# isxml/YOLO-SOMI

Measured on AMD Instinct MI355X. Metric: images/sec train (forward+loss+backward+Adam+EMA) @640, VisDrone-shaped synthetic, yolov5l-SOMI (DCNv3 blocks), higher is better.
Workload: dtype f32; 1 GPU; yolov5l-SOMI (DCNv3 blocks) training step: uint8 ingest + forward (batch-stat BN) + ComputeLoss + backward + Adam + EMA, 640x640, batch 32/GPU (BASELINE configs[1] shape); batch_per_gpu=32, imgsz=640, params=77918970, classes=10, parallelism=dp1

## Files before the change

### include/somi_hip.h

```cpp
#ifndef SOMI_HIP_H
#define SOMI_HIP_H

#include <stddef.h>
#include <stdint.h>

#ifdef __cplusplus
extern "C" {
#endif

#define SOMI_ABI_VERSION 15

#define SOMI_EINVAL   (-1)
#define SOMI_ENOTIMPL (-2)
#define SOMI_EWORKSPACE (-3)

typedef void *somi_stream_t;

int somi_abi_version(void);
const char *somi_last_error(void);
size_t somi_sizeof_desc(int which);

enum somi_act { SOMI_ACT_NONE = 0, SOMI_ACT_SILU = 1, SOMI_ACT_GELU = 2, SOMI_ACT_RELU = 3, SOMI_ACT_SIGMOID = 4,
                SOMI_ACT_LEAKY = 5 ,
                SOMI_ACT_HSWISH = 6  };
// ... 326 lines not shown

int somi_detect_decode_f32(const float *box, int box_cs, const float *cls, int cls_cs, const float *anchors_px_host,
                           float stride, float *raw, float *z, int B, int ny, int nx, int na, int nc, int total,
                           int row_off, somi_stream_t stream);

int somi_red_nchunk(long npix);
int somi_bn_stats_nhwc_f32(const float *x, int x_cs, int x_coff, long npix, int C, float eps, float momentum,
                           const float *gamma, const float *beta, float *mean, float *rstd, float *scale, float *shift,
                           float *running_mean, float *running_var, float *workspace, somi_stream_t stream);
int somi_bn_stats_act_nhwc_f32(const float *x, int x_cs, int x_coff, int act, long npix, int C, float eps, float momentum,
                               const float *gamma, const float *beta, float *mean, float *rstd, float *scale, float *shift,
                               float *running_mean, float *running_var, float *workspace, somi_stream_t stream);
int somi_bn_stats_partials_f32(const float *part_sum, const float *part_sumsq, int rows, long npix, int C, float eps, float momentum,
                               const float *gamma, const float *beta, float *mean, float *rstd, float *scale, float *shift,
                               float *running_mean, float *running_var, float *workspace, somi_stream_t stream);
int somi_bn_local_sums_f64(const float *x, int x_cs, int x_coff, long npix, int C, const float *pivot , const float *part_sum,
                           const float *part_sumsq, int rows, double *sums, float *workspace, somi_stream_t stream);
int somi_bn_stats_from_sums_f64(const double *all_sums, int nranks, int C, float eps, float momentum, const float *gamma, const float *beta,
                                float *mean, float *rstd, float *scale, float *shift, float *running_mean, float *running_var,
                                somi_stream_t stream);
int somi_bn_act_backward_sums_f64(const float *dz, int dz_cs, int dz_coff, const float *x, int x_cs, int x_coff, const float *mean,
                                  const float *scale, const float *shift, int act, int order, long npix, int C, double *sums, float *workspace,
                                  somi_stream_t stream);
int somi_bn_act_backward_apply_sync_f32(const float *dz, int dz_cs, int dz_coff, const float *x, int x_cs, int x_coff, const float *mean,
                                        const float *rstd, const float *scale, const float *shift, int act, int order,
                                        const double *local_sums, const double *all_sums, int nranks, float *dx, int dx_cs, int dx_coff,
                                        float *dgamma, float *dbeta, long npix, int C, float *workspace, somi_stream_t stream);
int somi_chan_affine_act_nhwc_f32(const float *x, int x_cs, int x_coff, const float *scale, const float *shift, int act,
                                  int order, float *z, int z_cs, int z_coff, long npix, int C, const float *residual ,
                                  int res_cs, int res_coff, somi_stream_t stream);
// ... 55 lines not shown
                        float *db, float *dx, int ldx_out, int dx_accumulate, float *workspace, int B, int nin, int nout,
                        somi_stream_t stream);
int somi_odconv_synth_f32(const float *attn, const float *Wk, const float *biask, float *wout, float *bout, int B, int Cin, int Cin_pad,
                          int Cout, int kk, int K, somi_stream_t stream);
size_t somi_odconv_synth_bwd_workspace_floats(int B, int Cin, int Cout, int kk, int K);
int somi_odconv_synth_bwd_f32(const float *dWb, const float *attn, const float *Wk, const float *biask, const float *dbias_b, float *dWk,
                              float *dbiask, float *dattn, float *workspace, int B, int Cin, int Cin_pad, int Cout, int kk, int K,
                              somi_stream_t stream);

int somi_adam_ema_step_f32(float *param, const float *grad, float *exp_avg, float *exp_avg_sq, float *ema, long n, float lr, float beta1,
                           float beta2, float eps, float weight_decay, int step, float ema_decay, somi_stream_t stream);
int somi_sgd_ema_step_f32(float *param, const float *grad, float *momentum_buf, float *ema, long n, float lr, float momentum,
                          float weight_decay, int step, float ema_decay, somi_stream_t stream);
int somi_axpby_f32(float *y, const float *x, long n, float a, float b, somi_stream_t stream);
int somi_pack_dgrad_weights_f32(const float *w_packed, float *w_dgrad, int Cout, int taps, int Cin, somi_stream_t stream);

int somi_gconv2d_stat_rows(int B, int Ho, int Wo, int Cw);
int somi_gconv2d_nhwc_f32(const float *x, int x_cs, int x_coff, int B, int H, int W, int C1, const float *w, int w_cs, const float *bias,
                          int groups, int k, int stride, float *y, int y_cs, int y_coff, int C2, int Cw, int act, const float *residual,
                          int res_cs, int res_coff, float *stat_sum, float *stat_sumsq, const float *stat_pivot, somi_stream_t stream);
int somi_gconv2d_dgrad_nhwc_f32(const float *dy, int dy_cs, int dy_coff, int B, int Ho, int Wo, int C2, const float *w, int w_cs, int groups,
                                int k, int stride, float *dx, int dx_cs, int dx_coff, int H, int W, int C1, int Cx, const float *acc1,
                                int acc1_cs, int acc1_coff, const float *acc2, int acc2_cs, int acc2_coff, somi_stream_t stream);
size_t somi_gconv2d_wgrad_workspace_floats(int B, int Ho, int Wo, int C2, int cin_g, int k);
int somi_gconv2d_wgrad_nhwc_f32(const float *x, int x_cs, int x_coff, int B, int H, int W, int C1, const float *dy, int dy_cs, int dy_coff,
                                int Ho, int Wo, int C2, int groups, int k, int stride, float *dw, int accumulate, float *workspace,
                                size_t workspace_floats, somi_stream_t stream);

int somi_dwlk_strip_length(void);
int somi_dwlk_strips_per_workgroup(int B, int H, int W, int C, int wgrad);
// ... 162 lines not shown
```

### yolo-somi_amd/csrc/optim.hip

```cpp
#include "common.h"

namespace somi {

typedef float f32x4 __attribute__((ext_vector_type(4)));

__global__ __launch_bounds__(256) void adam_ema_kernel(float *__restrict__ p, const float *__restrict__ g, float *__restrict__ m, float *__restrict__ v,
                                                       float *__restrict__ ema, long n, float lr, float b1, float b2, float eps, float wd,
                                                       float bc1, float bc2_sqrt, float ema_d) {
    const float step = lr / bc1;
    const long n4 = n >> 2;
    for (long i = blockIdx.x * 256L + threadIdx.x; i < n4; i += (long)gridDim.x * 256) {
        f32x4 pv = *reinterpret_cast<f32x4 *>(p + i * 4);
        f32x4 gv = *reinterpret_cast<const f32x4 *>(g + i * 4) + wd * pv;
        f32x4 mv = b1 * *reinterpret_cast<f32x4 *>(m + i * 4) + (1.f - b1) * gv;
        f32x4 vv = b2 * *reinterpret_cast<f32x4 *>(v + i * 4) + (1.f - b2) * gv * gv;
#pragma unroll
        for (int e = 0; e < 4; ++e) pv[e] -= step * mv[e] / (sqrtf(vv[e]) / bc2_sqrt + eps);
        *reinterpret_cast<f32x4 *>(p + i * 4) = pv;
        *reinterpret_cast<f32x4 *>(m + i * 4) = mv;
        *reinterpret_cast<f32x4 *>(v + i * 4) = vv;
        if (ema) *reinterpret_cast<f32x4 *>(ema + i * 4) = ema_d * *reinterpret_cast<f32x4 *>(ema + i * 4) + (1.f - ema_d) * pv;
    }
    for (long i = n4 * 4 + blockIdx.x * 256L + threadIdx.x; i < n; i += (long)gridDim.x * 256) {
        float pv = p[i];
// ... 15 lines not shown
        p[i] = pv;
        buf[i] = bv;
        if (ema) ema[i] = ema_d * ema[i] + (1.f - ema_d) * pv;
    }
}

__global__ __launch_bounds__(256) void axpby_kernel(float *__restrict__ y, const float *__restrict__ x, long n, float a, float b) {
    for (long i = blockIdx.x * 256L + threadIdx.x; i < n; i += (long)gridDim.x * 256) y[i] = a * y[i] + b * x[i];
}

static inline int grid_for(long n) {
    long g = (n / 4 + 255) / 256;
    return (int)(g < 1 ? 1 : (g > 4096 ? 4096 : g));
}

__global__ __launch_bounds__(256) void pack_dgrad_kernel(const float *__restrict__ w, float *__restrict__ wt, int Cout, int T, int Cin) {
    __shared__ float tile[32][33];
    const int t = blockIdx.z, co0 = blockIdx.y * 32, ci0 = blockIdx.x * 32;
    const int tx = threadIdx.x & 31, ty = threadIdx.x >> 5;
    for (int r = ty; r < 32; r += 8) {
        const int co = co0 + r, ci = ci0 + tx;
        tile[r][tx] = (co < Cout && ci < Cin) ? w[((size_t)co * T + t) * Cin + ci] : 0.f;
    }
    __syncthreads();
    for (int r = ty; r < 32; r += 8) {
        const int ci = ci0 + r, co = co0 + tx;
        if (ci < Cin && co < Cout) wt[((size_t)ci * T + t) * Cout + co] = tile[tx][r];
    }
}

}

using namespace somi;

extern "C" int somi_adam_ema_step_f32(float *param, const float *grad, float *exp_avg, float *exp_avg_sq, float *ema, long n, float lr, float beta1,
                                      float beta2, float eps, float weight_decay, int step, float ema_decay, somi_stream_t stream) {
    SOMI_REQUIRE(param && grad && exp_avg && exp_avg_sq && n > 0 && step >= 1, SOMI_EINVAL, "adam: bad arguments");
    SOMI_REQUIRE(aligned16(param) && aligned16(grad) && aligned16(exp_avg) && aligned16(exp_avg_sq) && (!ema || aligned16(ema)), SOMI_EINVAL,
                 "adam: segments must be 16 B aligned");
    const float bc1 = 1.f - powf(beta1, (float)step), bc2 = 1.f - powf(beta2, (float)step);
    hipLaunchKernelGGL(adam_ema_kernel, dim3(grid_for(n)), dim3(256), 0, (hipStream_t)stream, param, grad, exp_avg, exp_avg_sq, ema, n, lr, beta1,
                       beta2, eps, weight_decay, bc1, sqrtf(bc2), ema_decay);
    return launch_status("somi_adam_ema_step_f32");
// ... 8 lines not shown
}

extern "C" int somi_axpby_f32(float *y, const float *x, long n, float a, float b, somi_stream_t stream) {
    SOMI_REQUIRE(y && x && n > 0, SOMI_EINVAL, "axpby: bad arguments");
    hipLaunchKernelGGL(axpby_kernel, dim3(grid_for(n * 4)), dim3(256), 0, (hipStream_t)stream, y, x, n, a, b);
    return launch_status("somi_axpby_f32");
}

extern "C" int somi_pack_dgrad_weights_f32(const float *w_packed, float *w_dgrad, int Cout, int taps, int Cin, somi_stream_t stream) {
    using namespace somi;
    SOMI_REQUIRE(w_packed && w_dgrad && Cout > 0 && taps > 0 && Cin > 0 && taps < 65536, SOMI_EINVAL, "pack dgrad: bad arguments");
    hipLaunchKernelGGL(pack_dgrad_kernel, dim3(cdiv(Cin, 32), cdiv(Cout, 32), taps), dim3(256), 0, (hipStream_t)stream, w_packed, w_dgrad,
                       Cout, taps, Cin);
    return launch_status("somi_pack_dgrad_weights_f32");
}
```

### yolo-somi_amd/csrc/train_ops.hip

```cpp
#include "common.h"

namespace somi {
typedef int i32x4_ __attribute__((ext_vector_type(4)));

typedef float f32x4 __attribute__((ext_vector_type(4)));

static inline int red_chunk(long npix) {
    long c = (npix + 1023) / 1024;
    c = (c + 31) / 32 * 32;
    return (int)(c < 32 ? 32 : (c > 4096 ? 4096 : c));
}

__device__ __forceinline__ float act_fwd(float u, int act) { return apply_act_rt(u, act); }
__device__ __forceinline__ float act_grad(float u, int act) {
    switch (act) {
        case SOMI_ACT_SILU: { const float s = 1.f / (1.f + expf(-u)); return s * (1.f + u * (1.f - s)); }
        case SOMI_ACT_GELU: return 0.5f * (1.f + erff(u * 0.70710678118654752440f)) + u * 0.39894228040143267794f * expf(-0.5f * u * u);
        case SOMI_ACT_RELU: return u > 0.f ? 1.f : 0.f;
        case SOMI_ACT_SIGMOID: { const float s = 1.f / (1.f + expf(-u)); return s * (1.f - s); }
        case SOMI_ACT_LEAKY: return u > 0.f ? 1.f : 0.1f;
        case SOMI_ACT_HSWISH: return u <= -3.f ? 0.f : (u >= 3.f ? 1.f : (2.f * u + 3.f) * (1.f / 6.f));
        default: return 1.f;
    }
}
// ... 21 lines not shown
            for (long p = p0 + rr; p < p1; p += rows_par) f(p, (cq0 + cq) * 4, s1, s2);
        }
        l1[threadIdx.x] = s1;
        l2[threadIdx.x] = s2;
        __syncthreads();
        if (threadIdx.x < ncq) {
            for (int r2 = 1; r2 < rows_par; ++r2) { s1 += l1[r2 * ncq + cq]; s2 += l2[r2 * ncq + cq]; }
            const long o = (long)chunk * C + (cq0 + cq) * 4;
            *reinterpret_cast<f32x4 *>(part1 + o) = s1;
            *reinterpret_cast<f32x4 *>(part2 + o) = s2;
        }
        __syncthreads();
    }
}

constexpr int S2_CH = 4, S2_GRP = 256 / S2_CH;
__device__ __forceinline__ bool stage2_sums(const float *__restrict__ p1, const float *__restrict__ p2, int nchunk, int C, int &c, double &s1, double &s2) {
    __shared__ double l1[256], l2[256];
    const int cl = threadIdx.x % S2_CH, grp = threadIdx.x / S2_CH;
    c = blockIdx.x * S2_CH + cl;
    double a0 = 0.0, a1 = 0.0, b0 = 0.0, b1 = 0.0;
    if (c < C) {
        constexpr int S2_DEEP = 8;
        for (int k = grp; k < nchunk; k += S2_DEEP * S2_GRP) {
            float v[S2_DEEP], w[S2_DEEP];
#pragma unroll
            for (int j = 0; j < S2_DEEP; ++j) {
                const int r = k + j * S2_GRP;
                const bool ok = r < nchunk;
                v[j] = ok ? p1[(long)r * C + c] : 0.f;
                w[j] = (ok && p2) ? p2[(long)r * C + c] : 0.f;
            }
#pragma unroll
            for (int j = 0; j < S2_DEEP; j += 2) { a0 += v[j]; a1 += v[j + 1]; b0 += w[j]; b1 += w[j + 1]; }
        }
    }
    l1[threadIdx.x] = a0 + a1;
    l2[threadIdx.x] = b0 + b1;
    __syncthreads();
    if (grp != 0 || c >= C) return false;
    double t1 = 0.0, t2 = 0.0;
#pragma unroll
    for (int g = 0; g < S2_GRP; ++g) { t1 += l1[g * S2_CH + cl]; t2 += l2[g * S2_CH + cl]; }
    s1 = t1;
    s2 = t2;
    return true;
// ... 26 lines not shown
    double var = q / (double)npix - dm * dm;
    if (var < 0.0) var = 0.0;
    const float rs = (float)(1.0 / sqrt(var + (double)eps));
    mean[c] = (float)m;
    rstd[c] = rs;
    const float g = gamma ? gamma[c] : 1.f, b = beta ? beta[c] : 0.f;
    scale[c] = g * rs;
    shift[c] = b - (float)m * g * rs;
    if (running_mean) {
        const double unb = npix > 1 ? var * (double)npix / (double)(npix - 1) : var;
        running_mean[c] = (1.f - momentum) * running_mean[c] + momentum * (float)m;
        running_var[c] = (1.f - momentum) * running_var[c] + momentum * (float)unb;
    }
}

__global__ __launch_bounds__(256) void rows_fold_kernel(const float *__restrict__ p1, const float *__restrict__ p2, int rows, int C, int per,
                                                        float *__restrict__ o1, float *__restrict__ o2) {
    const int c = blockIdx.y * 256 + threadIdx.x;
    if (c >= C) return;
    const int r0 = blockIdx.x * per, r1 = min(r0 + per, rows);
    float a = 0.f, b = 0.f;
    for (int r = r0; r < r1; ++r) { a += p1[(size_t)r * C + c]; b += p2[(size_t)r * C + c]; }
    o1[(size_t)blockIdx.x * C + c] = a;
    o2[(size_t)blockIdx.x * C + c] = b;
}

__global__ __launch_bounds__(256) void sums_fold_f64_kernel(const float *__restrict__ p1, const float *__restrict__ p2, int nchunk, int C, long npix,
                                                            double *__restrict__ sums, const float *__restrict__ pivot, int central) {
    int c;
    double s1, s2;
    if (blockIdx.x == 0 && threadIdx.x == 0) sums[2 * (size_t)C] = (double)npix;
    if (!stage2_sums(p1, p2, nchunk, C, c, s1, s2)) return;
    if (central) {
        const double dm = s1 / (double)npix;
        double m2 = s2 - s1 * dm;
        sums[c] = (pivot ? (double)pivot[c] : 0.0) + dm;
        sums[(size_t)C + c] = m2 < 0.0 ? 0.0 : m2;
// ... 386 lines not shown
            }
        }
#pragma unroll
        for (int j = 0; j < 7; ++j) {
            lr[threadIdx.x] = acc[j];
            __syncthreads();
            if (threadIdx.x < ncq) {
                f32x4 t = acc[j];
                for (int r2 = 1; r2 < rows_par; ++r2) t += lr[r2 * ncq + cq];
                *reinterpret_cast<f32x4 *>(part + j * plane + row * C + c) = t;
            }
            __syncthreads();
        }
    }
}
__global__ __launch_bounds__(256) void cbam_bn_bwd_stage2(const float *__restrict__ part, int rows, int nimg, int C, int HW, const float *__restrict__ davg,
                                                          const float *__restrict__ dmax, const float *__restrict__ rstd,
                                                          const float *__restrict__ scale, float *__restrict__ coefA, float *__restrict__ coefB,
                                                          float *__restrict__ coefC, float *dgamma, float *dbeta) {
    __shared__ double l1[256], l2[256];
    const int cl = threadIdx.x % S2_CH, grp = threadIdx.x / S2_CH;
    const int c = blockIdx.x * S2_CH + cl;
    const long plane = (long)rows * C;
    const float inv_hw = 1.f / (float)HW;
    double a1 = 0.0, a2 = 0.0;
    if (c < C) {
        for (int k = grp; k < rows; k += 4 * S2_GRP) {
            float v[4][6], ka[4], km[4];
#pragma unroll
            for (int j = 0; j < 4; ++j) {
                const int r = k + j * S2_GRP;
                const bool ok = r < rows;
                const int b = ok ? r / nimg : 0;
#pragma unroll
                for (int q = 0; q < 6; ++q) v[j][q] = ok ? part[(q + 1) * plane + (long)r * C + c] : 0.f;
                ka[j] = ok ? davg[(long)b * C + c] * inv_hw : 0.f;
                km[j] = ok ? dmax[(long)b * C + c] : 0.f;
            }
#pragma unroll
            for (int j = 0; j < 4; ++j) {
                a1 += (double)(v[j][0] + ka[j] * v[j][2] + km[j] * v[j][4]);
                a2 += (double)(v[j][1] + ka[j] * v[j][3] + km[j] * v[j][5]);
            }
        }
    }
    l1[threadIdx.x] = a1;
    l2[threadIdx.x] = a2;
    __syncthreads();
    if (grp != 0 || c >= C) return;
    double s1 = 0.0, s2 = 0.0;
#pragma unroll
    for (int g = 0; g < S2_GRP; ++g) { s1 += l1[g * S2_CH + cl]; s2 += l2[g * S2_CH + cl]; }
    const double rs = rstd[c], sc = scale[c], n = (double)rows / nimg * HW;
    const double D = rs * s2;
    coefA[c] = (float)sc;
    coefB[c] = (float)(-sc * rs * D / n);
    coefC[c] = (float)(-sc * s1 / n);
// ... 182 lines not shown
    SOMI_REQUIRE(!running_mean == !running_var, SOMI_EINVAL, "bn stats: running_mean and running_var go together");
    hipStream_t s = (hipStream_t)stream;
    const float *p1 = part_sum, *p2 = part_sumsq;
    int nchunk = rows;
    if (rows > 1024) {
        const int per = cdiv(rows, 1024);
        nchunk = cdiv(rows, per);
        float *o1 = workspace, *o2 = workspace + (size_t)1024 * C;
        hipLaunchKernelGGL(rows_fold_kernel, dim3(nchunk, cdiv(C, 256)), dim3(256), 0, s, part_sum, part_sumsq, rows, C, per, o1, o2);
        p1 = o1;
        p2 = o2;
    }
    hipLaunchKernelGGL(bn_stats_stage2, dim3(cdiv(C, S2_CH)), dim3(256), 0, s, p1, p2, nchunk, C, npix, eps, momentum, gamma, beta, mean, rstd,
                       scale, shift, running_mean, running_var);
    return launch_status("somi_bn_stats_partials_f32");
}

extern "C" int somi_chan_affine_act_nhwc_f32(const float *x, int x_cs, int x_coff, const float *scale, const float *shift, int act,
                                             int order, float *z, int z_cs, int z_coff, long npix, int C, const float *residual,
                                             int res_cs, int res_coff, somi_stream_t stream) {
    SOMI_REQUIRE_SLICES("chan affine act", {"x", x, x_cs, x_coff, C}, {"z", z, z_cs, z_coff, C}, {"residual", residual, res_cs, res_coff, C, kOptional});
    SOMI_REQUIRE(scale && shift && npix > 0 && C % 4 == 0 && (order == 0 || order == 1) && aligned16(scale) && aligned16(shift), SOMI_EINVAL,
                 "chan affine act: bad arguments");
    launch_affine_act(x, x_cs, x_coff, scale, shift, act, order, z, z_cs, z_coff, npix, C, residual, res_cs, res_coff, (hipStream_t)stream);
    return launch_status("somi_chan_affine_act_nhwc_f32");
}

extern "C" int somi_bn_act_backward_nhwc_f32(const float *dz, int dz_cs, int dz_coff, const float *x, int x_cs, int x_coff, const float *mean,
                                             const float *rstd, const float *scale, const float *shift, int act, int order,
                                             int batch_stats, float *dx, int dx_cs, int dx_coff, float *dgamma, float *dbeta, long npix,
// ... 191 lines not shown
```

### yolo-somi_amd/somi_amd/_lib.py

```python
import ctypes as C
import os

_HERE = os.path.dirname(os.path.abspath(__file__))
LIB_PATH = os.environ.get('SOMI_HIP_LIB') or os.path.join(os.path.dirname(_HERE), 'lib', 'libsomi_hip.so')

ABI_VERSION = 15
c_f32p = C.c_void_p
c_stream = C.c_void_p


class ConvDesc(C.Structure):
    _fields_ = [(n, C.c_void_p) for n in ('x', 'w', 'bias', 'post_scale', 'post_shift', 'residual', 'a_chan_scale',
                                          'a_pix_scale', 'y')] + \
               [(n, C.c_int32) for n in ('B', 'H', 'W', 'Cin', 'x_cs', 'x_coff', 'Ho', 'Wo', 'Cout', 'y_cs', 'y_coff',
                                         'kh', 'kw', 'stride', 'pad', 'dil', 'res_cs', 'res_coff', 'act', 'per_sample_w')] + \
               [('res2_cs', C.c_int32), ('res2_coff', C.c_int32), ('workspace', C.c_void_p), ('workspace_bytes', C.c_uint64),
                ('residual2', C.c_void_p), ('stat_sum', C.c_void_p), ('stat_sumsq', C.c_void_p), ('stat_pivot', C.c_void_p), ('prec', C.c_int32)]


class LossDesc(C.Structure):
    _fields_ = [('p', C.c_void_p * 4), ('grad', C.c_void_p * 4), ('ny', C.c_int32 * 4), ('nx', C.c_int32 * 4),
                ('nl', C.c_int32), ('na', C.c_int32), ('nc', C.c_int32), ('B', C.c_int32), ('nt', C.c_int32),
                ('targets', C.c_void_p), ('anchors', C.c_void_p), ('balance', C.c_float * 4),
                ('box_gain', C.c_float), ('obj_gain', C.c_float), ('cls_gain', C.c_float), ('cls_pw', C.c_float),
# ... 124 lines not shown
    'somi_global_pool_nhwc_f32': (I, [P, I, I, I, I, I, P, P, P, S]),
    'somi_global_pool_act_nhwc_f32': (I, [P, I, I, I, I, I, I, P, P, P, P, S]),
    'somi_affine_silu_pool_rows': (I, [I, I, I]),
    'somi_affine_silu_pool_nhwc_f32': (I, [P, I, I, P, P, P, I, I, I, I, I, P, P, P, S]),
    'somi_attn_mlp_f32': (I, [I, P, P, P, P, P, P, P, I, I, I, S]),
    'somi_chan_stats_nhwc_f32': (I, [P, I, I, P, P, I, I, I, S]),
    'somi_spatial_attn_f32': (I, [P, P, P, P, I, I, I, I, S]),
    'somi_cbam_apply_nhwc_f32': (I, [P, I, I, P, P, P, P, P, I, I, I, I, I, I, I, S]),
    'somi_scale_channels_nhwc_f32': (I, [P, P, P, P, I, I, I, S]),
    'somi_odconv_weights_f32': (I, [P] * 18 + [I] * 7 + [S]),
    'somi_detect_decode_f32': (I, [P, I, P, I, C.POINTER(C.c_float), F, P, P, I, I, I, I, I, I, I, S]),
    'somi_red_nchunk': (I, [C.c_long]),
    'somi_bn_stats_nhwc_f32': (I, [P, I, I, C.c_long, I, F, F, P, P, P, P, P, P, P, P, P, S]),
    'somi_bn_stats_act_nhwc_f32': (I, [P, I, I, I, C.c_long, I, F, F, P, P, P, P, P, P, P, P, P, S]),
    'somi_bn_stats_partials_f32': (I, [P, P, I, C.c_long, I, F, F, P, P, P, P, P, P, P, P, P, S]),
    'somi_bn_local_sums_f64': (I, [P, I, I, C.c_long, I, P, P, P, I, P, P, S]),
    'somi_bn_stats_from_sums_f64': (I, [P, I, I, F, F, P, P, P, P, P, P, P, P, S]),
    'somi_bn_act_backward_sums_f64': (I, [P, I, I, P, I, I, P, P, P, I, I, C.c_long, I, P, P, S]),
    'somi_bn_act_backward_apply_sync_f32': (I, [P, I, I, P, I, I, P, P, P, P, I, I, P, P, I, P, I, I, P, P, C.c_long, I, P, S]),
    'somi_chan_affine_act_nhwc_f32': (I, [P, I, I, P, P, I, I, P, I, I, C.c_long, I, P, I, I, S]),
    'somi_bn_act_backward_nhwc_f32': (I, [P, I, I, P, I, I, P, P, P, P, I, I, I, P, I, I, P, P, C.c_long, I, P, S]),
    'somi_bn_pooled_rows': (I, [I, I]),
    'somi_bn_act_backward_pooled_nhwc_f32': (I, [P, I, I, P, I, I, P, P, P, P, I, I, P, P, P, P, I, I, P, P, I, I, I, P, S]),
    'somi_add_nhwc_f32': (I, [P, I, I, P, I, I, P, I, I, C.c_long, I, S]),
    'somi_chan_sum_nhwc_f32': (I, [P, I, I, C.c_long, I, P, P, S]),
    'somi_img_nchunk': (I, [I]),
    'somi_cbam_bwd_pixel_argmax_f32': (I, [P, I, I, P, I, I, P, P, P, P, P, P, I, I, I, S]),
    'somi_cbam_bn_bwd_workspace_floats': (C.c_size_t, [I, I, I]),
    'somi_cbam_bn_bwd_reduce_f32': (I, [P, I, I, P, I, I, P, P, P, P, P, P, P, P, P, P, I, I, I, S]),
    'somi_cbam_bn_bwd_apply_f32': (I, [P, I, I, P, I, I, P, P, P, P, P, P, P, P, P, P, P, P, I, I, P, P, P, I, I, I, S]),
# ... 11 lines not shown
    'somi_tta_descale_f32': (I, [P, C.c_long, I, F, I, F, S]),
    'somi_sppf_pool_bwd_nhwc_f32': (I, [P, P, P, I, I, I, I, I, I, S]),
    'somi_sppf_pool_codes_nhwc_f32': (I, [P, P, I, I, I, I, I, I, S]),
    'somi_bifpn_bwd_nhwc_f32': (I, [C.POINTER(C.c_void_p), C.POINTER(C.c_void_p), C.POINTER(C.c_int), P, F, I, P, P, P, I, I, I, I, S]),
    'somi_dwconv3x3_bwd_workspace_floats': (Z, [I, I, I]),
    'somi_dwconv3x3_bwd_nhwc_f32': (I, [P, P, P, P, P, P, P, P, I, I, I, I, S]),
    'somi_scale_channels_bwd_nhwc_f32': (I, [P, P, P, P, P, P, I, I, I, S]),
    'somi_linear_f32': (I, [P, I, P, P, I, P, I, I, I, I, I, S]),
    'somi_linear_bwd_f32': (I, [P, I, P, P, P, I, I, I, P, P, P, I, I, P, I, I, I, S]),
    'somi_odconv_synth_f32': (I, [P, P, P, P, P, I, I, I, I, I, I, S]),
    'somi_odconv_synth_bwd_workspace_floats': (Z, [I, I, I, I, I]),
    'somi_odconv_synth_bwd_f32': (I, [P, P, P, P, P, P, P, P, P, I, I, I, I, I, I, S]),
    'somi_adam_ema_step_f32': (I, [P, P, P, P, P, C.c_long, F, F, F, F, F, I, F, S]),
    'somi_sgd_ema_step_f32': (I, [P, P, P, P, C.c_long, F, F, F, I, F, S]),
    'somi_pack_dgrad_weights_f32': (I, [P, P, I, I, I, S]),
    'somi_gconv2d_stat_rows': (I, [I, I, I, I]),
    'somi_gconv2d_nhwc_f32': (I, [P, I, I, I, I, I, I, P, I, P, I, I, I, P, I, I, I, I, I, P, I, I, P, P, P, S]),
    'somi_gconv2d_dgrad_nhwc_f32': (I, [P, I, I, I, I, I, I, P, I, I, I, I, P, I, I, I, I, I, I, P, I, I, P, I, I, S]),
    'somi_gconv2d_wgrad_workspace_floats': (Z, [I, I, I, I, I, I]),
    'somi_gconv2d_wgrad_nhwc_f32': (I, [P, I, I, I, I, I, I, P, I, I, I, I, I, I, I, I, P, I, P, Z, S]),
    'somi_dwlk_strip_length': (I, []),
    'somi_dwlk_strips_per_workgroup': (I, [I, I, I, I, I]),
    'somi_dwlk_stat_rows': (I, [I, I, I, I]),
    'somi_dwlk_nhwc_f32': (I, [Slice, P, I, P, I, I, P, P, Slice, Slice, I, I, I, I, P, P, P, S]),
    'somi_dwlk_dgrad_nhwc_f32': (I, [Slice, P, I, I, Slice, Slice, Slice, I, I, I, I, S]),
    'somi_dwlk_wgrad_workspace_floats': (Z, [I, I, I, I, I]),
    'somi_dwlk_wgrad_nhwc_f32': (I, [Slice, Slice, I, I, I, I, I, P, P, I, P, Z, S]),
    'somi_psa_attention_f32': (I, [P, I, I, I, I, I, P, I, I, P, P, S]),
    'somi_psa_attention_backward_f32': (I, [P, I, I, P, I, I, P, I, I, P, I, I, I, P, I, I, P, P, S]),
    'somi_swin_attention_lse_floats': (Z, [I, I, I, I]),
# ... 133 lines not shown
```

### yolo-somi_amd/somi_amd/blocks.py

```python
import math

import torch
import torch.nn as nn

from . import ops
from .pack import pack_conv_weight, pack_dgrad_weight, pack_gconv_weight, pad4, bn_fold


class Act:
    __slots__ = ('t', 'coff', 'c', 'up', 'pooled', 'pool')

    def __init__(self, t, coff=0, c=None, up=0):
        self.t, self.coff, self.c, self.up = t, coff, (t.shape[3] - coff if c is None else c), up
        self.pooled = None
        self.pool = None

    @property
    def shape(self):
        return self.t.shape

    def slice(self, coff, c):
        return Act(self.t, self.coff + coff, c)


# ... 215 lines not shown
            raise NotImplementedError('grouped / depthwise dilated Conv is not on the SOMI path (dense convs only)')
        if d != 1 and s != 1:
            raise NotImplementedError(f'dilated Conv with stride {s} is not on the SOMI path (its data gradient runs at stride 1 only)')
        if g != 1:
            if k not in (1, 3, 5) or s not in (1, 2) or autopad(k, p, d) != k // 2:
                raise NotImplementedError(f'grouped Conv with k={k}, s={s}, p={p} is not on the SOMI path (k 1/3/5, stride 1/2, pad k // 2)')
            if c1 % g == 0 and c1 // g > 16:
                raise NotImplementedError(f'grouped Conv with {c1 // g} input channels per group is not on the SOMI path (at most 16)')
        self.conv = nn.Conv2d(c1, c2, k, s, autopad(k, p, d), groups=g, dilation=d, bias=False)
        self.bn = nn.BatchNorm2d(c2)
        self.act = nn.SiLU() if act is True else (act if isinstance(act, nn.Module) else nn.Identity())

    accumulates = folds_pooled = True
    reduction = property(lambda self: self.conv.stride[0])

    def _pack(self, dev):
        if self.conv.groups > 1:
            return self._pack_grouped(dev)
        if self.training:
            w = self.conv.weight
            c2, c1, k = w.shape[0], w.shape[1], w.shape[2]
            cp, c1p = pad4(c2), pad4(c1)
            master = self.__dict__.get('_master')
            if master is not None and master[0].device == dev:
                wp, gp = master
                wt = ops.pack_dgrad_weights(wp, cp, k * k, c1p)
            else:
                wf = w.detach().float()
                wp, gp, wt = pack_conv_weight(wf, cout_pad=cp).to(dev), None, pack_dgrad_weight(wf).to(dev)
            return dict(wp=wp, gp=gp, wt=wt, **_bn_vectors(self.bn, dev, cp))
        return _pack_wb(*_fold_conv_bn(self.conv, getattr(self, 'bn', None)), dev)

    def _pack_grouped(self, dev):
        c2, cp = self.conv.out_channels, pad4(self.conv.out_channels)
        if not self.training:
            w, b = _fold_conv_bn(self.conv, getattr(self, 'bn', None))
            bp = torch.zeros(cp, device=dev)
            bp[:c2] = b.to(dev)
            return pack_gconv_weight(w, cp).to(dev), bp
        return dict(gw=pack_gconv_weight(self.conv.weight.detach(), cp).to(dev), **_bn_vectors(self.bn, dev, cp))

# ... 3458 lines not shown
```

### yolo-somi_amd/somi_amd/ops.py

```python
import ctypes as C
import math
import os

import torch

from . import _lib
from ._lib import ConvDesc, check

DCN_DIRECT = os.environ.get('SOMI_DCN_DIRECT', '0') == '1'
PROFILE = None



class _timed:
    __slots__ = ('info', 'ev')

    def __init__(self, info):
        self.info, self.ev = info, None

    def __enter__(self):
        if PROFILE is not None:
            self.ev = torch.cuda.Event(enable_timing=True), torch.cuda.Event(enable_timing=True)
            self.ev[0].record()

# ... 1578 lines not shown
    ws = torch.empty(2 * 1024 * c, device=dev, dtype=torch.float32)
    check(_lib.lib().somi_bn_stats_partials_f32(part[0].data_ptr(), part[1].data_ptr(), rows, npix, c, float(eps), float(momentum), _ptr(gamma),
                                                _ptr(beta), _ptr(mean), _ptr(rstd), _ptr(scale), _ptr(shift), _ptr(running_mean),
                                                _ptr(running_var), _ptr(ws), _stream()), 'bn_stats_partials')
    return mean, rstd, scale, shift


def chan_affine_act(x, c, x_coff, scale, shift, act, order, out, out_coff=0, residual=None, res_coff=0):
    check(_lib.lib().somi_chan_affine_act_nhwc_f32(_ptr(_f32c(x)), x.shape[3], x_coff, _ptr(scale), _ptr(shift), ACT[act], order,
                                                   _ptr(_f32c(out)), out.shape[3], out_coff, _npix(x), c,
                                                   _ptr(residual), residual.shape[3] if residual is not None else 0, res_coff,
                                                   _stream()), 'chan_affine_act')
    return out


def pack_dgrad_weights(w_packed, cout, taps, cin):
    out = torch.empty(cin, taps * cout, device=w_packed.device, dtype=torch.float32)
    check(_lib.lib().somi_pack_dgrad_weights_f32(_ptr(_f32c(w_packed)), _ptr(out), cout, taps, cin, _stream()), 'pack_dgrad_weights')
    return out


def bn_act_backward(dz, dz_coff, x, x_coff, c, mean, rstd, scale, shift, act, order, batch_stats, dx, dx_coff=0, dgamma=None,
                    dbeta=None, pooled=None):
    n = _npix(x)
    if pooled is not None:
        davg, dmax, amaxp = pooled
        if SYNC_BN is None and batch_stats and davg.shape[1] == c and x.dim() == 4:
            B, HW = x.shape[0], x.shape[1] * x.shape[2]
            L = _lib.lib()
            ws = torch.empty(2 * L.somi_bn_pooled_rows(B, HW) * c + 3 * ((c + 3) // 4 * 4), device=x.device, dtype=torch.float32)
            check(L.somi_bn_act_backward_pooled_nhwc_f32(_ptr(None if dz is None else _f32c(dz)), 0 if dz is None else dz.shape[3], dz_coff,
                                                         _ptr(_f32c(x)), x.shape[3], x_coff, _ptr(mean),
                                                         _ptr(rstd), _ptr(scale), _ptr(shift), ACT[act], order, _ptr(davg), _ptr(dmax),
                                                         _ptr(amaxp), _ptr(_f32c(dx)), dx.shape[3], dx_coff, _ptr(dgamma), _ptr(dbeta), B, HW, c,
# ... 181 lines not shown
```

### yolo-somi_amd/somi_amd/optim.py

```python
import math

import torch
import torch.nn as nn

from . import _lib
from ._lib import check
from .ops import _ptr, _stream


def reference_param_groups(model):
    g0, g1, g2 = [], [], []
    for v in model.modules():
        if hasattr(v, 'bias') and isinstance(v.bias, nn.Parameter):
            g2.append(v.bias)
        if isinstance(v, nn.BatchNorm2d):
            g0.append(v.weight)
        elif hasattr(v, 'weight') and isinstance(v.weight, nn.Parameter):
            g1.append(v.weight)
    return g0, g1, g2


class _Flat:

    def __init__(self, tensors, dev, packed=None):
# ... 35 lines not shown
        self.model = model
        g0, g1, g2 = reference_param_groups(model)
        idle = {id(p) for m in model.modules() for name in getattr(m, 'never_runs', ()) for p in getattr(m, name).parameters()}
        seen = set()
        groups = []
        for plist, wd in ((g0, 0.0), (g1, weight_decay), (g2, 0.0)):
            plist = [p for p in plist if id(p) not in idle and id(p) not in seen and not seen.add(id(p))]
            groups.append((plist, wd))
        self._ungrouped = [p for p in model.parameters() if id(p) not in seen]
        from .blocks import Conv
        from .pack import pad4
        owners = {id(m.conv.weight): m for m in model.modules() if isinstance(m, Conv) and m.conv.groups == 1}
        packed = {k: (pad4(m.conv.out_channels), m.conv.kernel_size[0], m.conv.kernel_size[1], pad4(m.conv.in_channels))
                  for k, m in owners.items()}
        self.param_groups, self._flat = [], []
        for plist, wd in groups:
            fp, fg = _Flat(plist, dev, packed), _Flat(plist, dev, packed)
            with torch.no_grad():
                for i, ((p, v), (_, gv)) in enumerate(zip(fp.views(), fg.views())):
                    v.copy_(p.data)
                    p.data = v
                    p.grad = gv
                    if fp.packed[i] is not None:
                        owners[id(p)].__dict__['_master'] = (fp.storage_of(i), fg.storage_of(i))
            st = dict(p=fp, g=fg, m=torch.zeros_like(fp.data), v=torch.zeros_like(fp.data),
                      ema=fp.data.clone() if ema else None)
            self._flat.append(st)
            grp = dict(params=plist, lr=lr, initial_lr=lr, betas=betas, eps=eps, weight_decay=wd)
            if self.sgd:
                grp.update(momentum=betas[0], nesterov=True)
            self.param_groups.append(grp)
        self._buf_owner = []
        for mod in model.modules():
            for name, b in mod._buffers.items():
                if b is not None and b.dtype.is_floating_point and b.numel() > 0 and b.device == dev:
                    self._buf_owner.append((mod, name))
        bufs = [getattr(mod, name) for mod, name in self._buf_owner]
        self._bflat = _Flat(bufs, dev)
        with torch.no_grad():
            for i, (mod, name) in enumerate(self._buf_owner):
                v = self._bflat.view_of(i)
                v.copy_(bufs[i])
                setattr(mod, name, v)
        self._bflat.tensors = [getattr(mod, name) for mod, name in self._buf_owner]
        self._buf_ema = self._bflat.data.clone() if ema else None
        self.ema_decay, self.updates, self.steps = ema_decay, 0, 0
        if hasattr(model, 'invalidate'):
            model.invalidate()

    @property
    def flat_params(self):
        return [st['p'].data for st in self._flat]

    @property
    def flat_buffers(self):
        return self._bflat.data[:self._bflat.n_pad]

    def reset_ema(self):
        for st in self._flat:
            if st['ema'] is not None:
                st['ema'].copy_(st['p'].data)
        if self._buf_ema is not None:
            self._buf_ema.copy_(self._bflat.data)
# ... 19 lines not shown
            if st['p'].n == 0:
                continue
            if self.sgd:
                check(L.somi_sgd_ema_step_f32(_ptr(st['p'].data), _ptr(st['g'].data), _ptr(st['m']), _ptr(st['ema']), st['p'].n_pad, float(grp['lr']),
                                              float(grp['momentum']), float(grp['weight_decay']), self.steps, float(d if d is not None else 0.0),
                                              _stream()), 'sgd_ema_step')
                continue
            check(L.somi_adam_ema_step_f32(_ptr(st['p'].data), _ptr(st['g'].data), _ptr(st['m']), _ptr(st['v']), _ptr(st['ema']), st['p'].n_pad,
                                           float(grp['lr']), float(grp['betas'][0]), float(grp['betas'][1]), float(grp['eps']),
                                           float(grp['weight_decay']), self.steps, float(d if d is not None else 0.0), _stream()), 'adam_ema_step')
        if d is not None and self._buf_ema is not None and self._bflat.n > 0:
            check(L.somi_axpby_f32(_ptr(self._buf_ema), _ptr(self._bflat.data), self._bflat.n_pad, float(d), float(1 - d), _stream()),
                  'ema buffers')
        if hasattr(self.model, 'invalidate'):
            self.model.invalidate()

    def ema_state_dict(self):
        sd = {k: v.detach().clone() for k, v in self.model.state_dict().items()}
        name_of = {id(p): n for n, p in self.model.named_parameters()}
        for st in self._flat:
            if st['ema'] is None:
                continue
            for i, p in enumerate(st['p'].tensors):
                sd[name_of[id(p)]] = st['p'].view_of(i, st['ema']).clone()
        if self._buf_ema is not None:
            mname = {id(m): n for n, m in self.model.named_modules()}
            for i, (mod, name) in enumerate(self._buf_owner):
                prefix = mname[id(mod)]
                sd[(prefix + '.' if prefix else '') + name] = self._bflat.view_of(i, self._buf_ema).clone()
        return sd
# ... 9 lines not shown
```

Measured before the change: 99.46 images/s.

## Batch dgrad weight repacking into one table-driven kernel after optimizer step

Adds a table-driven kernel that repacks the dgrad-transposed weights of all conv layers in a parameter group in one launch, writing into a persistent preallocated buffer. The optimizer calls it after each step, and conv modules reuse that buffer unless the weight version has changed, replacing many per-layer pack launches and allocations. Separately, the BN stats, rows-fold and CBAM backward stage-2 reductions now issue more loads up front (depth 16, clamped indices, sched barrier) for more memory-level parallelism, at the cost of higher register pressure. It also exposes several fold kernels through new C entry points.

```diff
diff --git a/include/somi_hip.h b/include/somi_hip.h
--- a/include/somi_hip.h
+++ b/include/somi_hip.h
@@ -364,6 +364,14 @@
 int somi_bn_stats_partials_f32(const float *part_sum, const float *part_sumsq, int rows, long npix, int C, float eps, float momentum,
                                const float *gamma, const float *beta, float *mean, float *rstd, float *scale, float *shift,
                                float *running_mean, float *running_var, float *workspace, somi_stream_t stream);
+int somi_rows_fold_f32(const float *p1, const float *p2, int rows, int C, int per, float *o1, float *o2, somi_stream_t stream);
+int somi_bn_stats_fold_f32(const float *p1, const float *p2, int rows, long npix, int C, float eps, float momentum, const float *gamma,
+                           const float *beta, float *mean, float *rstd, float *scale, float *shift, float *running_mean, float *running_var,
+                           somi_stream_t stream);
+int somi_bn_act_bwd_fold_f32(const float *p1, const float *p2, int rows, long npix, int C, const float *mean, const float *rstd, const float *scale,
+                             int batch_stats, float *coefA, float *coefB, float *coefC, float *dgamma, float *dbeta, somi_stream_t stream);
+int somi_cbam_bn_bwd_fold_f32(const float *part, int rows, int nimg, int C, int HW, const float *davg, const float *dmax, const float *rstd,
+                              const float *scale, float *coefA, float *coefB, float *coefC, float *dgamma, float *dbeta, somi_stream_t stream);
 int somi_bn_local_sums_f64(const float *x, int x_cs, int x_coff, long npix, int C, const float *pivot , const float *part_sum,
                            const float *part_sumsq, int rows, double *sums, float *workspace, somi_stream_t stream);
 int somi_bn_stats_from_sums_f64(const double *all_sums, int nranks, int C, float eps, float momentum, const float *gamma, const float *beta,
@@ -449,6 +457,9 @@
                           float weight_decay, int step, float ema_decay, somi_stream_t stream);
 int somi_axpby_f32(float *y, const float *x, long n, float a, float b, somi_stream_t stream);
 int somi_pack_dgrad_weights_f32(const float *w_packed, float *w_dgrad, int Cout, int taps, int Cin, somi_stream_t stream);
+#define SOMI_PACK_TABLE_COLS 6
+int somi_pack_dgrad_table_f32(const float *src, long src_floats, float *dst, long dst_floats, const int64_t *table, int n_layers, long total_tiles,
+                              somi_stream_t stream);
 
 int somi_gconv2d_stat_rows(int B, int Ho, int Wo, int Cw);
 int somi_gconv2d_nhwc_f32(const float *x, int x_cs, int x_coff, int B, int H, int W, int C1, const float *w, int w_cs, const float *bias,
diff --git a/yolo-somi_amd/csrc/optim.hip b/yolo-somi_amd/csrc/optim.hip
--- a/yolo-somi_amd/csrc/optim.hip
+++ b/yolo-somi_amd/csrc/optim.hip
@@ -53,9 +53,8 @@
     return (int)(g < 1 ? 1 : (g > 4096 ? 4096 : g));
 }
 
-__global__ __launch_bounds__(256) void pack_dgrad_kernel(const float *__restrict__ w, float *__restrict__ wt, int Cout, int T, int Cin) {
+__device__ __forceinline__ void pack_dgrad_tile(const float *__restrict__ w, float *__restrict__ wt, int Cout, int T, int Cin, int t, int co0, int ci0) {
     __shared__ float tile[32][33];
-    const int t = blockIdx.z, co0 = blockIdx.y * 32, ci0 = blockIdx.x * 32;
     const int tx = threadIdx.x & 31, ty = threadIdx.x >> 5;
     for (int r = ty; r < 32; r += 8) {
         const int co = co0 + r, ci = ci0 + tx;
@@ -66,6 +65,26 @@
         const int ci = ci0 + r, co = co0 + tx;
         if (ci < Cin && co < Cout) wt[((size_t)ci * T + t) * Cout + co] = tile[tx][r];
     }
+}
+__global__ __launch_bounds__(256) void pack_dgrad_kernel(const float *__restrict__ w, float *__restrict__ wt, int Cout, int T, int Cin) {
+    pack_dgrad_tile(w, wt, Cout, T, Cin, blockIdx.z, blockIdx.y * 32, blockIdx.x * 32);
+}
+
+constexpr int PT_COLS = SOMI_PACK_TABLE_COLS;
+__global__ __launch_bounds__(256) void pack_dgrad_table_kernel(const float *__restrict__ src, long src_floats, float *__restrict__ dst, long dst_floats,
+                                                               const int64_t *__restrict__ table, int n_layers) {
+    const long blk = blockIdx.x;
+    int lo = 0, hi = n_layers - 1;
+    while (lo < hi) {
+        const int mid = (lo + hi + 1) >> 1;
+        if (table[(long)mid * PT_COLS + 5] <= blk) lo = mid; else hi = mid - 1;
+    }
+    const int64_t *rec = table + (long)lo * PT_COLS;
+    const long so = rec[0], dofs = rec[1], Cout = rec[2], T = rec[3], Cin = rec[4], local = blk - rec[5];
+    if (so < 0 || dofs < 0 || Cout <= 0 || T <= 0 || Cin <= 0 || Cout > (1 << 20) || Cin > (1 << 20) || T > 65535 || local < 0) return;
+    const long n = Cout * T * Cin, tx = (Cin + 31) / 32, ty = (Cout + 31) / 32;
+    if (so + n > src_floats || dofs + n > dst_floats || local >= tx * ty * T) return;
+    pack_dgrad_tile(src + so, dst + dofs, (int)Cout, (int)T, (int)Cin, (int)(local / (tx * ty)), (int)(local / tx % ty) * 32, (int)(local % tx) * 32);
 }
 
 }
@@ -104,3 +123,13 @@
                        Cout, taps, Cin);
     return launch_status("somi_pack_dgrad_weights_f32");
 }
+
+extern "C" int somi_pack_dgrad_table_f32(const float *src, long src_floats, float *dst, long dst_floats, const int64_t *table, int n_layers,
+                                         long total_tiles, somi_stream_t stream) {
+    using namespace somi;
+    SOMI_REQUIRE(src && dst && table && src_floats > 0 && dst_floats > 0 && n_layers > 0 && total_tiles > 0 && total_tiles <= 0x7fffffffL, SOMI_EINVAL,
+                 "pack dgrad table: bad arguments");
+    hipLaunchKernelGGL(pack_dgrad_table_kernel, dim3((unsigned)total_tiles), dim3(256), 0, (hipStream_t)stream, src, src_floats, dst, dst_floats, table,
+                       n_layers);
+    return launch_status("somi_pack_dgrad_table_f32");
+}
diff --git a/yolo-somi_amd/csrc/train_ops.hip b/yolo-somi_amd/csrc/train_ops.hip
--- a/yolo-somi_amd/csrc/train_ops.hip
+++ b/yolo-somi_amd/csrc/train_ops.hip
@@ -59,22 +59,30 @@
     }
 }
 
-constexpr int S2_CH = 4, S2_GRP = 256 / S2_CH;
+constexpr int S2_CH = 4, S2_GRP = 256 / S2_CH, S2_DEEP = 16;
 __device__ __forceinline__ bool stage2_sums(const float *__restrict__ p1, const float *__restrict__ p2, int nchunk, int C, int &c, double &s1, double &s2) {
     __shared__ double l1[256], l2[256];
     const int cl = threadIdx.x % S2_CH, grp = threadIdx.x / S2_CH;
     c = blockIdx.x * S2_CH + cl;
     double a0 = 0.0, a1 = 0.0, b0 = 0.0, b1 = 0.0;
     if (c < C) {
-        constexpr int S2_DEEP = 8;
         for (int k = grp; k < nchunk; k += S2_DEEP * S2_GRP) {
             float v[S2_DEEP], w[S2_DEEP];
 #pragma unroll
+            for (int j = 0; j < S2_DEEP; ++j) v[j] = p1[(long)min(k + j * S2_GRP, nchunk - 1) * C + c];
+            if (p2) {
+#pragma unroll
+                for (int j = 0; j < S2_DEEP; ++j) w[j] = p2[(long)min(k + j * S2_GRP, nchunk - 1) * C + c];
+            } else {
+#pragma unroll
+                for (int j = 0; j < S2_DEEP; ++j) w[j] = 0.f;
+            }
+            __builtin_amdgcn_sched_barrier(0);
+#pragma unroll
             for (int j = 0; j < S2_DEEP; ++j) {
-                const int r = k + j * S2_GRP;
-                const bool ok = r < nchunk;
-                v[j] = ok ? p1[(long)r * C + c] : 0.f;
-                w[j] = (ok && p2) ? p2[(long)r * C + c] : 0.f;
+                const bool ok = k + j * S2_GRP < nchunk;
+                v[j] = ok ? v[j] : 0.f;
+                w[j] = (ok && p2) ? w[j] : 0.f;
             }
 #pragma unroll
             for (int j = 0; j < S2_DEEP; j += 2) { a0 += v[j]; a1 += v[j + 1]; b0 += w[j]; b1 += w[j + 1]; }
@@ -131,13 +139,29 @@
     }
 }
 
+constexpr int FOLD_DEEP = 16;
 __global__ __launch_bounds__(256) void rows_fold_kernel(const float *__restrict__ p1, const float *__restrict__ p2, int rows, int C, int per,
                                                         float *__restrict__ o1, float *__restrict__ o2) {
     const int c = blockIdx.y * 256 + threadIdx.x;
     if (c >= C) return;
     const int r0 = blockIdx.x * per, r1 = min(r0 + per, rows);
     float a = 0.f, b = 0.f;
-    for (int r = r0; r < r1; ++r) { a += p1[(size_t)r * C + c]; b += p2[(size_t)r * C + c]; }
+    for (int r = r0; r < r1; r += FOLD_DEEP) {
+        float v[FOLD_DEEP], w[FOLD_DEEP];
+#pragma unroll
+        for (int j = 0; j < FOLD_DEEP; ++j) {
+            const size_t o = (size_t)min(r + j, r1 - 1) * C + c;
+            v[j] = p1[o];
+            w[j] = p2[o];
+        }
+        __builtin_amdgcn_sched_barrier(0);
+#pragma unroll
+        for (int j = 0; j < FOLD_DEEP; ++j) {
+            const bool ok = r + j < r1;
+            a += ok ? v[j] : 0.f;
+            b += ok ? w[j] : 0.f;
+        }
+    }
     o1[(size_t)blockIdx.x * C + c] = a;
     o2[(size_t)blockIdx.x * C + c] = b;
 }
@@ -554,6 +578,7 @@
         }
     }
 }
+constexpr int CB_DEEP = 16;
 __global__ __launch_bounds__(256) void cbam_bn_bwd_stage2(const float *__restrict__ part, int rows, int nimg, int C, int HW, const float *__restrict__ davg,
                                                           const float *__restrict__ dmax, const float *__restrict__ rstd,
                                                           const float *__restrict__ scale, float *__restrict__ coefA, float *__restrict__ coefB,
@@ -565,22 +590,25 @@
     const float inv_hw = 1.f / (float)HW;
     double a1 = 0.0, a2 = 0.0;
     if (c < C) {
-        for (int k = grp; k < rows; k += 4 * S2_GRP) {
-            float v[4][6], ka[4], km[4];
-#pragma unroll
-            for (int j = 0; j < 4; ++j) {
-                const int r = k + j * S2_GRP;
-                const bool ok = r < rows;
-                const int b = ok ? r / nimg : 0;
-#pragma unroll
-                for (int q = 0; q < 6; ++q) v[j][q] = ok ? part[(q + 1) * plane + (long)r * C + c] : 0.f;
-                ka[j] = ok ? davg[(long)b * C + c] * inv_hw : 0.f;
-                km[j] = ok ? dmax[(long)b * C + c] : 0.f;
+        for (int k = grp; k < rows; k += CB_DEEP * S2_GRP) {
+            float v[CB_DEEP][6], ka[CB_DEEP], km[CB_DEEP];
+#pragma unroll
+            for (int j = 0; j < CB_DEEP; ++j) {
+                const int r = min(k + j * S2_GRP, rows - 1), b = r / nimg;
+#pragma unroll
+                for (int q = 0; q < 6; ++q) v[j][q] = part[(q + 1) * plane + (long)r * C + c];
+                ka[j] = davg[(long)b * C + c];
+                km[j] = dmax[(long)b * C + c];
             }
-#pragma unroll
-            for (int j = 0; j < 4; ++j) {
-                a1 += (double)(v[j][0] + ka[j] * v[j][2] + km[j] * v[j][4]);
-                a2 += (double)(v[j][1] + ka[j] * v[j][3] + km[j] * v[j][5]);
+            __builtin_amdgcn_sched_barrier(0);
+#pragma unroll
+            for (int j = 0; j < CB_DEEP; ++j) {
+                const bool ok = k + j * S2_GRP < rows;
+                const float kav = ka[j] * inv_hw;
+                const float t1 = __builtin_fmaf(km[j], v[j][4], __builtin_fmaf(kav, v[j][2], v[j][0]));
+                const float t2 = __builtin_fmaf(km[j], v[j][5], __builtin_fmaf(kav, v[j][3], v[j][1]));
+                a1 += ok ? (double)t1 : 0.0;
+                a2 += ok ? (double)t2 : 0.0;
             }
         }
     }
@@ -793,6 +821,43 @@
     hipLaunchKernelGGL(bn_stats_stage2, dim3(cdiv(C, S2_CH)), dim3(256), 0, s, p1, p2, nchunk, C, npix, eps, momentum, gamma, beta, mean, rstd,
                        scale, shift, running_mean, running_var);
     return launch_status("somi_bn_stats_partials_f32");
+}
+
+extern "C" int somi_rows_fold_f32(const float *p1, const float *p2, int rows, int C, int per, float *o1, float *o2, somi_stream_t stream) {
+    SOMI_REQUIRE(p1 && p2 && o1 && o2 && rows > 0 && C > 0 && per > 0, SOMI_EINVAL, "rows fold: bad arguments");
+    SOMI_REQUIRE(cdiv(C, 256) <= 65535, SOMI_EINVAL, "rows fold: C beyond the grid's y range");
+    hipLaunchKernelGGL(rows_fold_kernel, dim3(cdiv(rows, per), cdiv(C, 256)), dim3(256), 0, (hipStream_t)stream, p1, p2, rows, C, per, o1, o2);
+    return launch_status("somi_rows_fold_f32");
+}
+
+extern "C" int somi_bn_stats_fold_f32(const float *p1, const float *p2, int rows, long npix, int C, float eps, float momentum, const float *gamma,
+                                      const float *beta, float *mean, float *rstd, float *scale, float *shift, float *running_mean,
+                                      float *running_var, somi_stream_t stream) {
+    SOMI_REQUIRE(p1 && p2 && rows > 0 && npix > 0 && C > 0 && mean && rstd && scale && shift, SOMI_EINVAL, "bn stats fold: bad arguments");
+    SOMI_REQUIRE(!running_mean == !running_var, SOMI_EINVAL, "bn stats: running_mean and running_var go together");
+    hipLaunchKernelGGL(bn_stats_stage2, dim3(cdiv(C, S2_CH)), dim3(256), 0, (hipStream_t)stream, p1, p2, rows, C, npix, eps, momentum, gamma, beta, mean,
+                       rstd, scale, shift, running_mean, running_var);
+    return launch_status("somi_bn_stats_fold_f32");
+}
+
+extern "C" int somi_bn_act_bwd_fold_f32(const float *p1, const float *p2, int rows, long npix, int C, const float *mean, const float *rstd,
+                                        const float *scale, int batch_stats, float *coefA, float *coefB, float *coefC, float *dgamma, float *dbeta,
+                                        somi_stream_t stream) {
+    SOMI_REQUIRE(p1 && p2 && rows > 0 && npix > 0 && C > 0 && mean && rstd && scale && coefA && coefB && coefC, SOMI_EINVAL,
+                 "bn act backward fold: bad arguments");
+    hipLaunchKernelGGL(bn_act_bwd_stage2, dim3(cdiv(C, S2_CH)), dim3(256), 0, (hipStream_t)stream, p1, p2, rows, C, npix, mean, rstd, scale, batch_stats,
+                       coefA, coefB, coefC, dgamma, dbeta);
+    return launch_status("somi_bn_act_bwd_fold_f32");
+}
+
+extern "C" int somi_cbam_bn_bwd_fold_f32(const float *part, int rows, int nimg, int C, int HW, const float *davg, const float *dmax, const float *rstd,
+                                         const float *scale, float *coefA, float *coefB, float *coefC, float *dgamma, float *dbeta,
+                                         somi_stream_t stream) {
+    SOMI_REQUIRE(part && rows > 0 && nimg > 0 && rows % nimg == 0 && C > 0 && HW > 0 && davg && dmax && rstd && scale && coefA && coefB && coefC,
+                 SOMI_EINVAL, "cbam bn backward fold: bad arguments");
+    hipLaunchKernelGGL(cbam_bn_bwd_stage2, dim3(cdiv(C, S2_CH)), dim3(256), 0, (hipStream_t)stream, part, rows, nimg, C, HW, davg, dmax, rstd, scale, coefA,
+                       coefB, coefC, dgamma, dbeta);
+    return launch_status("somi_cbam_bn_bwd_fold_f32");
 }
 
 extern "C" int somi_chan_affine_act_nhwc_f32(const float *x, int x_cs, int x_coff, const float *scale, const float *shift, int act,
diff --git a/yolo-somi_amd/somi_amd/_lib.py b/yolo-somi_amd/somi_amd/_lib.py
--- a/yolo-somi_amd/somi_amd/_lib.py
+++ b/yolo-somi_amd/somi_amd/_lib.py
@@ -162,6 +162,10 @@
     'somi_bn_stats_nhwc_f32': (I, [P, I, I, C.c_long, I, F, F, P, P, P, P, P, P, P, P, P, S]),
     'somi_bn_stats_act_nhwc_f32': (I, [P, I, I, I, C.c_long, I, F, F, P, P, P, P, P, P, P, P, P, S]),
     'somi_bn_stats_partials_f32': (I, [P, P, I, C.c_long, I, F, F, P, P, P, P, P, P, P, P, P, S]),
+    'somi_rows_fold_f32': (I, [P, P, I, I, I, P, P, S]),
+    'somi_bn_stats_fold_f32': (I, [P, P, I, C.c_long, I, F, F, P, P, P, P, P, P, P, P, S]),
+    'somi_bn_act_bwd_fold_f32': (I, [P, P, I, C.c_long, I, P, P, P, I, P, P, P, P, P, S]),
+    'somi_cbam_bn_bwd_fold_f32': (I, [P, I, I, I, I, P, P, P, P, P, P, P, P, P, S]),
     'somi_bn_local_sums_f64': (I, [P, I, I, C.c_long, I, P, P, P, I, P, P, S]),
     'somi_bn_stats_from_sums_f64': (I, [P, I, I, F, F, P, P, P, P, P, P, P, P, S]),
     'somi_bn_act_backward_sums_f64': (I, [P, I, I, P, I, I, P, P, P, I, I, C.c_long, I, P, P, S]),
@@ -203,6 +207,7 @@
     'somi_adam_ema_step_f32': (I, [P, P, P, P, P, C.c_long, F, F, F, F, F, I, F, S]),
     'somi_sgd_ema_step_f32': (I, [P, P, P, P, C.c_long, F, F, F, I, F, S]),
     'somi_pack_dgrad_weights_f32': (I, [P, P, I, I, I, S]),
+    'somi_pack_dgrad_table_f32': (I, [P, C.c_long, P, C.c_long, P, I, C.c_long, S]),
     'somi_gconv2d_stat_rows': (I, [I, I, I, I]),
     'somi_gconv2d_nhwc_f32': (I, [P, I, I, I, I, I, I, P, I, P, I, I, I, P, I, I, I, I, I, P, I, I, P, P, P, S]),
     'somi_gconv2d_dgrad_nhwc_f32': (I, [P, I, I, I, I, I, I, P, I, I, I, I, P, I, I, I, I, I, I, P, I, I, P, I, I, S]),
diff --git a/yolo-somi_amd/somi_amd/blocks.py b/yolo-somi_amd/somi_amd/blocks.py
--- a/yolo-somi_amd/somi_amd/blocks.py
+++ b/yolo-somi_amd/somi_amd/blocks.py
@@ -253,6 +253,10 @@
     accumulates = folds_pooled = True
     reduction = property(lambda self: self.conv.stride[0])
 
+    def invalidate(self):
+        super().invalidate()
+        self.__dict__.pop('_wt_current', None)
+
     def _pack(self, dev):
         if self.conv.groups > 1:
             return self._pack_grouped(dev)
@@ -263,7 +267,12 @@
             master = self.__dict__.get('_master')
             if master is not None and master[0].device == dev:
                 wp, gp = master
-                wt = ops.pack_dgrad_weights(wp, cp, k * k, c1p)
+                wt = self.__dict__.get('_master_wt')
+                if wt is None:
+                    wt = ops.pack_dgrad_weights(wp, cp, k * k, c1p)
+                elif self.__dict__.get('_wt_current') != w._version:
+                    ops.pack_dgrad_weights(wp, cp, k * k, c1p, out=wt)
+                    self.__dict__['_wt_current'] = w._version
             else:
                 wf = w.detach().float()
                 wp, gp, wt = pack_conv_weight(wf, cout_pad=cp).to(dev), None, pack_dgrad_weight(wf).to(dev)
diff --git a/yolo-somi_amd/somi_amd/ops.py b/yolo-somi_amd/somi_amd/ops.py
--- a/yolo-somi_amd/somi_amd/ops.py
+++ b/yolo-somi_amd/somi_amd/ops.py
@@ -1616,10 +1616,35 @@
     return out
 
 
-def pack_dgrad_weights(w_packed, cout, taps, cin):
-    out = torch.empty(cin, taps * cout, device=w_packed.device, dtype=torch.float32)
+def pack_dgrad_weights(w_packed, cout, taps, cin, out=None):
+    if out is None:
+        out = torch.empty(cin, taps * cout, device=w_packed.device, dtype=torch.float32)
+    elif tuple(out.shape) != (cin, taps * cout) or not out.is_contiguous() or out.dtype != torch.float32 or out.device != w_packed.device:
+        raise ValueError('pack_dgrad_weights: out must be a contiguous fp32 (cin, taps*cout) tensor on the weights\' device')
     check(_lib.lib().somi_pack_dgrad_weights_f32(_ptr(_f32c(w_packed)), _ptr(out), cout, taps, cin, _stream()), 'pack_dgrad_weights')
     return out
+
+
+PACK_TABLE_COLS = 6
+
+
+def pack_dgrad_table_rows(layers):
+    rows, first = [], 0
+    for src_off, dst_off, cout, taps, cin in layers:
+        rows.append([int(src_off), int(dst_off), int(cout), int(taps), int(cin), first])
+        first += int(taps) * ((int(cin) + 31) // 32) * ((int(cout) + 31) // 32)
+    return torch.tensor(rows, dtype=torch.int64).view(-1, PACK_TABLE_COLS), first
+
+
+def pack_dgrad_table(src, dst, table, total_tiles):
+    for t in (src, dst):
+        if t.dtype != torch.float32 or not t.is_contiguous() or t.device != table.device:
+            raise ValueError('pack_dgrad_table: src / dst must be contiguous fp32 tensors on the table\'s device')
+    if table.dtype != torch.int64 or table.dim() != 2 or table.shape[1] != PACK_TABLE_COLS or not table.is_contiguous():
+        raise ValueError('pack_dgrad_table: table must be a contiguous int64 (n, PACK_TABLE_COLS) tensor')
+    check(_lib.lib().somi_pack_dgrad_table_f32(_ptr(src), src.numel(), _ptr(dst), dst.numel(), _ptr(table), table.shape[0], int(total_tiles),
+                                               _stream()), 'pack_dgrad_table')
+    return dst
 
 
 def bn_act_backward(dz, dz_coff, x, x_coff, c, mean, rstd, scale, shift, act, order, batch_stats, dx, dx_coff=0, dgamma=None,
diff --git a/yolo-somi_amd/somi_amd/optim.py b/yolo-somi_amd/somi_amd/optim.py
--- a/yolo-somi_amd/somi_amd/optim.py
+++ b/yolo-somi_amd/somi_amd/optim.py
@@ -3,7 +3,7 @@
 import torch
 import torch.nn as nn
 
-from . import _lib
+from . import _lib, ops
 from ._lib import check
 from .ops import _ptr, _stream
 
@@ -73,8 +73,10 @@
         packed = {k: (pad4(m.conv.out_channels), m.conv.kernel_size[0], m.conv.kernel_size[1], pad4(m.conv.in_channels))
                   for k, m in owners.items()}
         self.param_groups, self._flat = [], []
+        self._repack = []
         for plist, wd in groups:
             fp, fg = _Flat(plist, dev, packed), _Flat(plist, dev, packed)
+            layers, mods, wt_n = [], [], 0
             with torch.no_grad():
                 for i, ((p, v), (_, gv)) in enumerate(zip(fp.views(), fg.views())):
                     v.copy_(p.data)
@@ -82,6 +84,16 @@
                     p.grad = gv
                     if fp.packed[i] is not None:
                         owners[id(p)].__dict__['_master'] = (fp.storage_of(i), fg.storage_of(i))
+                        cp, kh, kw, c1p = fp.packed[i]
+                        layers.append((fp.offsets[i], wt_n, cp, kh * kw, c1p))
+                        mods.append(owners[id(p)])
+                        wt_n += (cp * kh * kw * c1p + 127) // 128 * 128
+            if layers:
+                wt = torch.zeros(wt_n, device=dev, dtype=torch.float32)
+                for (_, o, cp, taps, c1p), m in zip(layers, mods):
+                    m.__dict__['_master_wt'] = wt[o:o + cp * taps * c1p].view(c1p, taps * cp)
+                table, tiles = ops.pack_dgrad_table_rows(layers)
+                self._repack.append((fp.data, wt, table.to(dev), tiles, mods))
             st = dict(p=fp, g=fg, m=torch.zeros_like(fp.data), v=torch.zeros_like(fp.data),
                       ema=fp.data.clone() if ema else None)
             self._flat.append(st)
@@ -106,6 +118,13 @@
         self.ema_decay, self.updates, self.steps = ema_decay, 0, 0
         if hasattr(model, 'invalidate'):
             model.invalidate()
+        self.repack_dgrad()
+
+    def repack_dgrad(self):
+        for src, wt, table, tiles, mods in self._repack:
+            ops.pack_dgrad_table(src, wt, table, tiles)
+            for m in mods:
+                m.__dict__['_wt_current'] = m.conv.weight._version
 
     @property
     def flat_params(self):
@@ -155,6 +174,7 @@
                   'ema buffers')
         if hasattr(self.model, 'invalidate'):
             self.model.invalidate()
+        self.repack_dgrad()
 
     def ema_state_dict(self):
         sd = {k: v.detach().clone() for k, v in self.model.state_dict().items()}
```

Measured after the change: 99.88 images/s, median of 6. Within noise of the previous version (+0.4%).
